# RM-Zhang/SGCDet

Hardware: AMD Instinct MI355X
Metric: scenes/sec (40-view ScanNet volume) at 1/2/4/8 MI355X; mAP@0.25 parity (higher is better)
Workload: dtype f32 (neck/head conv: 3xbf16-split MFMA, fp32 accumulate, ~1e-5 of fp32; wide 3x3x3 stride-1 layers through a Winograd F(2,3) transform along z: <= 2e-5 of the tensor scale per layer against the direct fp32 convolution); 1 GPU; cfg2_scannet: 40 views x 256 ch, images 256x320, FPN maps 64x80/32x40/16x20, D=12, voxels 40x40x16, top-k [800, 6400], neck 3-scale -> ScanNetImVoxelHeadV2; occupancy=predicted, masked_tail=False, input_layout=nchw, scenes_in_flight_per_gpu=4, launch=one hipGraph replay per scene (device-side pair counts, no host read-back)

## Files before the change

### include/sgcdet_amd_image.h

```cpp
#ifndef SGCDET_AMD_IMAGE_H_
#define SGCDET_AMD_IMAGE_H_

#include "sgcdet_amd.h"

#ifdef __cplusplus
extern "C" {
#endif

#define SGC_CONV2D_RELU 1
#define SGC_CONV2D_RELU_AFTER_ADD 2

int sgc_conv2d_nhwc_ex_bf16x3(const float *x, const uint16_t *w_hi, const uint16_t *w_lo, const float *scale,
                              const float *shift, const float *residual_or_null, float *y, int N, int H, int W, int Cin,
                              int Cout, int ksize, int stride, int transposed, int flags, int ldy, int col0, int ldr,
                              int softmax_cols, sgc_stream_t stream);
int sgc_conv2d_nhwc_ex_supported(int N, int H, int W, int Cin, int Cout, int ksize, int stride, int transposed, int ldy,
                                 int col0, int ldr , int softmax_cols);

int sgc_conv2d_stem7_bf16x3(const float *img, const uint16_t *w_hi, const uint16_t *w_lo, const float *scale,
                            const float *shift, float *y, int N, int H, int W, int relu, sgc_stream_t stream);

int sgc_nchw_to_nhwc_padc(const float *src, float *dst, int N, int C, int H, int W, int Cp, sgc_stream_t stream);

#ifdef __cplusplus
}
#endif
#endif
```

### sgcdet_amd/_abi.py

```python
import ctypes as C

_p = C.c_void_p
_i = C.c_int
_f = C.c_float
_d = C.c_double

SIGNATURES = {
    "sgc_depth_score_forward": [_p, _p, _p, _p, _p] + [_i] * 7 + [_p],
    "sgc_wms_forward": [_p, _p, _p, _p, _p, _p, _p] + [_i] * 7 + [_p],
    "sgc_wms_backward": [_p] * 11 + [_i] * 7 + [_p],
    "sgc_depth_score_backward": [_p] * 7 + [_i] * 7 + [_p],
    "sgc_dfa3d_forward": [_p] * 8 + [_i] * 9 + [_p],
    "sgc_dfa3d_backward": [_p] * 11 + [_i] * 9 + [_p],
    "sgc_dfa3d_forward_items": [_p] * 9 + [_i] * 9 + [_p],
    "sgc_dfa3d_backward_items": [_p] * 12 + [_i] * 9 + [_p],
    "sgc_dfa3d_backward_binned": [_p] * 11 + [_i] * 13 + [_p],
    "sgc_project_points": [_p] * 6 + [_i, _i, _f, _f, _f, _f, _p],
    "sgc_compact_pairs": [_p, _i, _i] + [_p] * 9 + [_p],
    "sgc_pairs_geometry_sample": [_p] * 7 + [_i] * 9 + [_p],
    "sgc_pairs_geometry_linear_bf16x3": [_p] * 11 + [_i] * 10 + [_p],
    "sgc_pairs_deform_gather": [_p] * 9 + [_i] * 12 + [_p],
    "sgc_depth_pairs": [_p, _p] + [_i] * 5 + [_p],
    "sgc_bin_pairs": [_p] * 9 + [_i] * 7 + [_p],
    "sgc_pairs_deform_gather_tiled": [_p, _i] + [_p] * 6 + [_i] * 15 + [_p],
# ... 61 lines not shown
    "sgc_linear_rows_blockdiag_supported": (C.c_int, [_i] * 3),
    "sgc_pairs_geometry_linear_workspace_bytes": (C.c_int64, [_i]),
}

TRAIN_SIGNATURES = {
    "sgc_plane_sweep_corr_backward": [_p] * 7 + [C.c_int64] + [_i] * 6 + [_p],
    "sgc_grad_sqnorm_batch": [_p, _i, _i, _p, _p, _p],
    "sgc_adamw_step_batch": [_p, _i, _i, _p, _i, _p, _f, _p],
    "sgc_head_loss_forward": [_p, _i] + [_p] * 4 + [_i] * 4 + [_d] * 5 + [_p] * 5 + [C.c_int64, _p],
    "sgc_head_loss_finalize": [_p, C.c_int64, _p, _i, _p] + [_d] * 3 + [_p] * 3,
    "sgc_head_loss_scale_grads": [_p, _p, _p] + [_i] * 3 + [_p] * 5,
}

TRAIN_INTROSPECTION = {
    "sgc_plane_sweep_corr_backward_workspace_bytes": (C.c_int64, [_i] * 5),
    "sgc_grad_sqnorm_batch_workspace_bytes": (C.c_int64, [_i]),
    "sgc_head_loss_workspace_bytes": (C.c_int64, [_i] * 2),
}

IMAGE_SIGNATURES = {
    "sgc_conv2d_nhwc_ex_bf16x3": [_p] * 7 + [_i] * 13 + [_p],
    "sgc_conv2d_stem7_bf16x3": [_p] * 6 + [_i] * 4 + [_p],
    "sgc_nchw_to_nhwc_padc": [_p, _p] + [_i] * 5 + [_p],
}

IMAGE_INTROSPECTION = {
    "sgc_conv2d_nhwc_ex_supported": (C.c_int, [_i] * 12),
}

CONV2D_RELU, CONV2D_RELU_AFTER_ADD = 1, 2


class OptimGroup(C.Structure):
    _fields_ = [("lr", C.c_double), ("weight_decay", C.c_double), ("beta1", C.c_double), ("beta2", C.c_double), ("eps", C.c_double)]


OPTIM_ITEM_BYTES = 64
HEAD_LOSS_LEVEL_BYTES = 64
HEAD_LOSS_MAX_SCALES = 4

ABI_VERSION = 4


class SgcError(RuntimeError):
    """Raised when an entry point returns a negative status."""


class Library:

    def __init__(self, path, train=False, image=False):
# ... 40 lines not shown
```

### sgcdet_amd/csrc/rows_gemm.hip

```cpp
#include <stdlib.h>

#include "conv_common.hpp"
#include "tuning.hpp"
#include "mma.hpp"
#include "diag.hpp"

namespace sgc {



struct RowsGemmParams {
  const float *x;
  int64_t ldx;
  const __bf16 *w_hi, *w_lo;
  const float *scale, *shift;
  const float *residual;
  void *y;
  const int32_t *m_dev;
  int M, N;
  int relu;
  int hm_S, hm_cm, hm_bf16;
  int ncg;
  int diag;
  unsigned long long *stamps;
  int64_t y_bytes;
  float *zero_row;
  const float *gw;
  const int32_t *go;
  int64_t x_rows;
};

constexpr int RG_ROWS = 32;

typedef unsigned int u32x4 __attribute__((ext_vector_type(4)));
constexpr unsigned RG_OOB = 0xfffffff0u;

template <int K, int NW, int DEPTH, int EPI, int NP = 3, bool GATHER = false>
__global__ __launch_bounds__(NW * 64, 2) void rows_gemm_bf16x3_kernel(const RowsGemmParams p) {
  static_assert(!GATHER || (DEPTH == 1 && EPI == 0), "the gather form runs the lockstep schedule with the plain epilogue");
  constexpr int NT = NW * 64;
  constexpr int KS = K / 16;
  constexpr int K4 = K / 4;
  constexpr int CH = RG_ROWS * K4 / NT;
  constexpr int PITCH = K + 8;
  constexpr int PLANE = RG_ROWS * PITCH;
  static_assert(RG_ROWS * K4 % NT == 0, "tile must deal evenly");
  extern __shared__ __attribute__((aligned(16))) unsigned char rg_smem[];
  __bf16 *lds = reinterpret_cast<__bf16 *>(rg_smem);

  const int tid = threadIdx.x, lane = tid & 63, wid = tid >> 6;
  const int fr = lane & 31, fh = lane >> 5;
  if (p.zero_row && blockIdx.x == 0)
    for (int c = tid; c < p.N; c += NT) p.zero_row[c] = 0.f;
  const int Mrows = p.m_dev ? min(p.M, *p.m_dev) : p.M;
  const int ntiles = (Mrows + RG_ROWS - 1) / RG_ROWS;
  const int xcd = blockIdx.x & 7, loc = blockIdx.x >> 3;
  const int cg = loc % p.ncg, stripe = (loc / p.ncg) * 8 + xcd, nstripes = gridDim.x / p.ncg;
  if (stripe >= ntiles) return;
  const int col = (cg * NW + wid) * 32 + fr;

  const __amdgpu_buffer_rsrc_t xr = __builtin_amdgcn_make_buffer_rsrc(
      const_cast<float *>(p.x), 0, (p.diag & 2) ? 0 : (int)(unsigned)((int64_t)(GATHER ? p.x_rows : Mrows) * p.ldx * 4), 0x00020000);
  const __amdgpu_buffer_rsrc_t gwr = __builtin_amdgcn_make_buffer_rsrc(const_cast<float *>(GATHER ? p.gw : p.x), 0,
                                                                        GATHER ? (int)(unsigned)((int64_t)Mrows * 16) : 0, 0x00020000);
  const __amdgpu_buffer_rsrc_t gor = __builtin_amdgcn_make_buffer_rsrc(const_cast<int32_t *>(GATHER ? p.go : (const int32_t *)p.x), 0,
                                                                        GATHER ? (int)(unsigned)((int64_t)Mrows * 16) : 0, 0x00020000);
  const __amdgpu_buffer_rsrc_t yr = __builtin_amdgcn_make_buffer_rsrc(
      p.y, 0, (p.diag & 1) ? 0 : (int)(unsigned)((EPI == 1 || EPI == 3) ? p.y_bytes : (int64_t)Mrows * p.N * 4), 0x00020000);
  const __amdgpu_buffer_rsrc_t rr = __builtin_amdgcn_make_buffer_rsrc(
      const_cast<float *>(EPI == 2 ? p.residual : p.x), 0, (int)(unsigned)(EPI == 2 ? (int64_t)Mrows * p.N * 4 : 0), 0x00020000);

  bf16x8 bh[KS], bl[KS];
  {
    const __bf16 *wh = p.w_hi + (int64_t)col * K + fh * 8, *wl = p.w_lo + (int64_t)col * K + fh * 8;
#pragma unroll
    for (int kk = 0; kk < KS; ++kk) {
      bh[kk] = *reinterpret_cast<const bf16x8 *>(wh + kk * 16);
      if constexpr (NP == 3) bl[kk] = *reinterpret_cast<const bf16x8 *>(wl + kk * 16);
    }
  }
  const float sc = p.scale ? p.scale[col] : 1.f, sh = p.shift ? p.shift[col] : 0.f;
  const bool relu = p.relu != 0, relu1 = p.relu == 1, relu2 = p.relu == 2;

  constexpr bool STAG = DEPTH == 0;
  static_assert(!STAG || NW == 8, "the staggered form pairs waves w and w + 4 of an 8-wave workgroup");
  constexpr int NTL = STAG ? NT / 2 : NT, RL = STAG ? RG_ROWS / 2 : RG_ROWS;
  static_assert(NTL % K4 == 0 && RL * K4 / NTL == CH, "chunks of a thread must share their column");
  const int late = STAG ? __builtin_amdgcn_readfirstlane(wid >> 2) : 0;
  const int tl = STAG ? (tid & (NTL - 1)) : tid;
  const int ld_row = tl / K4 + late * RL, ld_c4 = tl % K4;
  constexpr int TV = GATHER ? 4 * CH + CH : CH;
  auto load_tile = [&](int t, float4 (&ra)[TV]) {
    int ldx4 = (int)p.ldx * 4;
    asm volatile("" : "+s"(ldx4));
    if constexpr (GATHER) {
#pragma unroll
      for (int i = 0; i < CH; ++i) {
        const unsigned doff = t < ntiles ? (unsigned)(t * RG_ROWS + ld_row + i * (NTL / K4)) * 16u : RG_OOB;
        const u32x4 o = __builtin_amdgcn_raw_buffer_load_b128(gor, doff, 0, 0);
        const u32x4 w = __builtin_amdgcn_raw_buffer_load_b128(gwr, doff, 0, 0);
        ra[4 * CH + i] = make_float4(__uint_as_float(w[0]), __uint_as_float(w[1]), __uint_as_float(w[2]), __uint_as_float(w[3]));
#pragma unroll
        for (int k = 0; k < 4; ++k) {
          const u32x4 v = __builtin_amdgcn_raw_buffer_load_b128(xr, o[k] * (unsigned)ldx4 + ld_c4 * 16, 0, 0);
          ra[4 * i + k] = make_float4(__uint_as_float(v[0]), __uint_as_float(v[1]), __uint_as_float(v[2]), __uint_as_float(v[3]));
        }
      }
      return;
    }
    const unsigned base = t < ntiles ? (unsigned)(t * RG_ROWS + ld_row) * (unsigned)ldx4 + ld_c4 * 16 : RG_OOB;
#pragma unroll
    for (int i = 0; i < CH; ++i) {
      const u32x4 v = __builtin_amdgcn_raw_buffer_load_b128(xr, t < ntiles ? base + i * (NTL / K4) * ldx4 : RG_OOB, 0, 0);
      ra[i] = make_float4(__uint_as_float(v[0]), __uint_as_float(v[1]), __uint_as_float(v[2]), __uint_as_float(v[3]));
    }
  };
  auto split_tile = [&](const float4 (&ra)[TV], int buf) {
    __bf16 *a_hi = lds + buf * 2 * PLANE, *a_lo = a_hi + PLANE;
#pragma unroll
    for (int i = 0; i < CH; ++i) {
      const int row = ld_row + i * (NTL / K4), c4 = ld_c4;
      float v[4];
      if constexpr (GATHER) {
        const float wk[4] = {ra[4 * CH + i].x, ra[4 * CH + i].y, ra[4 * CH + i].z, ra[4 * CH + i].w};
        v[0] = v[1] = v[2] = v[3] = 0.f;
#pragma unroll
        for (int k = 0; k < 4; ++k) {
          v[0] = __builtin_fmaf(wk[k], ra[4 * i + k].x, v[0]); v[1] = __builtin_fmaf(wk[k], ra[4 * i + k].y, v[1]);
          v[2] = __builtin_fmaf(wk[k], ra[4 * i + k].z, v[2]); v[3] = __builtin_fmaf(wk[k], ra[4 * i + k].w, v[3]);
        }
      } else {
        v[0] = ra[i].x; v[1] = ra[i].y; v[2] = ra[i].z; v[3] = ra[i].w;
      }
      bf16x4 h, l;
#pragma unroll
      for (int e = 0; e < 4; ++e) {
        const __bf16 hb = op_hi<NP>(v[e]);
        h[e] = hb;
        l[e] = op_lo<NP>(v[e], hb);
      }
      *reinterpret_cast<bf16x4 *>(a_hi + row * PITCH + c4 * 4) = h;
// ... 405 lines not shown
  {
    static const bool diag_ok = getenv("SGC_DIAG") && atoi(getenv("SGC_DIAG")) == 1;
    p.diag = diag_ok ? g_tune_rows_diag : 0;
  }
  RG_STAMP_BIND(p);
  const int nw = (N % 256 == 0) ? 8 : 4;
  p.ncg = N / (nw * 32);
  const int cap_tiles = ceil_div(M, RG_ROWS);
  const int per_cu = nw == 8 ? 1 : 2;
  int stripes = device_cus() * per_cu / p.ncg;
  if (g_tune_rows_cu_pct > 0 && g_tune_rows_cu_pct < 100) stripes = stripes * g_tune_rows_cu_pct / 100;
  if (stripes > cap_tiles) stripes = cap_tiles;
  stripes = (stripes + 7) / 8 * 8;
  const int grid = stripes * p.ncg;
  const int depth = nw == 8 ? g_tune_rows_depth : 1;
  if (K == 256) {
    if (nw == 8) return depth == 0 ? launch_rows_gemm<256, 8, 0>(p, grid, st) : depth == 2 ? launch_rows_gemm<256, 8, 2>(p, grid, st) : launch_rows_gemm<256, 8, 1>(p, grid, st);
    return launch_rows_gemm<256, 4, 1>(p, grid, st);
  }
  if (nw == 8) return depth == 0 ? launch_rows_gemm<128, 8, 0>(p, grid, st) : depth == 2 ? launch_rows_gemm<128, 8, 2>(p, grid, st) : launch_rows_gemm<128, 8, 1>(p, grid, st);
  return launch_rows_gemm<128, 4, 1>(p, grid, st);
}

}

#if defined(SGC_RG_STAMPS)
extern "C" void sgc_diag_rows_stamp_buffer(unsigned long long *buf) { sgc::g_rows_stamp_buf = buf; }
#endif
```

### sgcdet_amd/plugin/conv_plan.py

```python
import os

import torch

from .. import ext

_PAD = 32

CONV_MODE = "bf16x3"
CONV_PRODUCTS = 3


def set_conv_mode(mode):
    global CONV_MODE, CONV_PRODUCTS
    if mode not in ("bf16x3", "f32", "bf16", "fp16"):
        raise ValueError(mode)
    CONV_MODE = "bf16x3" if mode in ("bf16", "fp16") else mode
    CONV_PRODUCTS = {"bf16": 1, "fp16": 2}.get(mode, 3)
    import torch
    if torch.cuda.is_available():
        ext.ops().lib.call("sgc_set_conv_products", CONV_PRODUCTS)


WINOGRAD_Z = {"0": False, "1": True}.get(os.environ.get("SGC_WINOGRAD_Z", ""), "auto")
WINOGRAD_Z_MIN_CH = int(os.environ.get("SGC_WINOGRAD_Z_MIN_CH", "256"))
# ... 268 lines not shown
        self.w_hi, self.w_lo = ext.ops().split_operand(wp)
        self.shift = torch.zeros(cout_p, dtype=torch.float32, device=w.device)
        if bias is not None:
            self.shift[:cout] = bias.detach().float()
        self.cout, self.cout_p = cout, cout_p

    def __call__(self, x, extra_zero_row=False, count=None):
        M = x.shape[0]
        if CONV_MODE == "bf16x3" and self.cout_p == self.cout:
            return ext.ops().linear_rows_bf16x3(x, self.w_hi, self.w_lo, self.shift, count=count, useful=self.useful,
                                                zero_tail=bool(extra_zero_row) and M > 0)
        if count is not None:
            raise NotImplementedError("device-side row counts need the bf16x3 path and out_features % 4 == 0")
        if CONV_MODE == "bf16x3":
            y, _ = ext.ops().conv3d_cl_bf16x3(x, self.w_hi, self.w_lo, (M, 1, 1), 1, 1, False, None, self.shift)
        else:
            y, _ = ext.ops().conv3d_cl(x, self.wt, (M, 1, 1), 1, 1, False, None, self.shift)
        return y if self.cout_p == self.cout else y[:, :self.cout]

    def headmajor(self, x, N, S, M, out_dtype=torch.float32):
        if CONV_MODE != "bf16x3" or self.cout_p != self.cout:
            raise NotImplementedError("head-major output needs the bf16x3 path and out_features % 4 == 0")
        return ext.ops().linear_rows_headmajor_bf16x3(x, self.w_hi, self.w_lo, self.shift, N, S, M, out_dtype=out_dtype)
```

### sgcdet_amd/plugin/voxformer.py

```python
import copy
import math
import warnings

import torch
import torch.nn as nn
import torch.nn.functional as F

from ..mmcv_lite import (ATTENTION, TRANSFORMER, TRANSFORMER_LAYER, TRANSFORMER_LAYER_SEQUENCE,
                         BaseModule, ModuleList, TransformerLayerSequence,
                         build_attention, build_feedforward_network, build_norm_layer,
                         build_transformer_layer_sequence, constant_init, xavier_init)
from ..functions import MultiScale3DDeformableAttnFunction_fp32
from .. import ext
from .conv_plan import BlockDiagSpec, LinearSpec, cached_plan, module_fingerprint


def _ops():
    return ext.ops()


TILED_GATHER = dict(enabled=True, min_pixels=2048, storage="f32",
                    cm32=dict(bin=(16, 22), halo=(3, 3), depth_in_lds=False),
                    cm16=dict(bin=(16, 22), halo=(3, 3), depth_in_lds=True))


GEO_LINEAR_FUSED = __import__("os").environ.get("SGC_GEO_LINEAR", "1") != "0"

TRAIN_BWD_TILED = dict(enabled=True, bin=(8, 22), halo=(2, 2))


def _tiled_env_overrides():
    import os
    if "SGC_TILED" in os.environ:
        TILED_GATHER["enabled"] = os.environ["SGC_TILED"] != "0"
    if os.environ.get("SGC_STORAGE") in ("f32", "bf16"):
        TILED_GATHER["storage"] = os.environ["SGC_STORAGE"]
    spec = os.environ.get("SGC_TRAIN_BWD")
    if spec == "0":
        TRAIN_BWD_TILED["enabled"] = False
    elif spec:
        bw, bh, hx, hy = (int(v) for v in spec.split(","))
        TRAIN_BWD_TILED.update(enabled=True, bin=(bw, bh), halo=(hx, hy))
    for key in ("cm32", "cm16"):
        spec = os.environ.get("SGC_TILED_" + key.upper())
        if spec:
            bw, bh, hx, hy, dl = (int(v) for v in spec.split(","))
            TILED_GATHER[key] = dict(bin=(bw, bh), halo=(hx, hy), depth_in_lds=bool(dl))


# ... 209 lines not shown
        wqo = w[:C] @ self.output_proj.weight.detach().double()
        bqo = w[:C] @ self.output_proj.bias.detach().double() + b[:C]
        wk, wv, bv = w[C:2 * C], w[2 * C:], b[2 * C:]
        scale = (1.0 / hd) ** 0.5
        wqp = torch.cat([scale * wk[h * hd:(h + 1) * hd].t() @ wqo[h * hd:(h + 1) * hd] for h in range(Hn)], 0)
        bqp = torch.cat([scale * wk[h * hd:(h + 1) * hd].t() @ bqo[h * hd:(h + 1) * hd] for h in range(Hn)], 0)
        wbd = torch.zeros((C, Hn * C), dtype=torch.float64, device=w.device)
        for h in range(Hn):
            wbd[h * hd:(h + 1) * hd, h * C:(h + 1) * C] = wv[h * hd:(h + 1) * hd]
        vg = None
        if self.projected_query_blockdiag and BlockDiagSpec.supported(Hn, C, hd):
            vg = BlockDiagSpec(wv.view(Hn, hd, C).float(), bv.float())
        return dict(qp=LinearSpec(wqp.float(), bqp.float()), vbd=LinearSpec(wbd.float(), bv.float(), useful=1.0 / Hn), vbd_g=vg)

    def _use_projected_query(self, gemm, n_views, n_rows_cap=0):
        if gemm is None or gemm.get("qp") is None or self.projected_query is False:
            return False
        if 2 * n_rows_cap * self.attention_pooling.num_heads * self.embed_dims * 4 > self.projected_query_max_bytes:
            return False
        if not _ops().view_attend_pq_supported(n_views, self.embed_dims, self.attention_pooling.num_heads):
            return False
        return self.projected_query is True or n_views >= self.projected_query_min_views

    def _forward_pairs(self, query, feat, dist, ref_cam, mask_u8, H, W, zero_query=False, static_counts=False, want_ctx=False):
        ops = _ops()
        C = self.embed_dims
        N, Nq = mask_u8.shape
        from .conv_plan import CONV_MODE
        use_mfma = self.deformable_attn and self.inter_view_aggregation == "attn" and C % 32 == 0
        pc = ops.compact_pairs(mask_u8)
        if static_counts:
            if not (use_mfma and CONV_MODE == "bf16x3"):
                raise NotImplementedError("static_counts needs the bf16x3 GEMM path (attn aggregation, C % 32 == 0)")
            n_pairs, n_valid = -1, Nq
            totals, pairs_cnt, valid_cnt = pc["totals"], pc["totals"][0:1], pc["totals"][1:2]
        else:
            n_pairs, n_valid, _, _ = pc["totals"].tolist()
            totals = pairs_cnt = valid_cnt = None
        if n_pairs == 0:
            if want_ctx:
                return torch.zeros((1, C), dtype=feat.dtype, device=feat.device), pc["row_of"]
            out = torch.zeros((1, Nq, C), dtype=feat.dtype, device=feat.device)
            return out if zero_query else self.dropout(out) + query
        pair_cam, pair_q = pc["pair_cam"], pc["pair_q"]
        gemm = self._gemm_plan() if use_mfma else None
        da = self.deformable_attention
        S = feat.shape[1]
        Cm = C // da.num_heads
        tiled = None
        if (self.deformable_attn and use_mfma and CONV_MODE in ("bf16x3", "f32") and TILED_GATHER["enabled"] and da.num_levels == 1
                and da.num_points == 4 and Cm in (16, 32) and TILED_GATHER["min_pixels"] <= H * W < 32767
                and dist.shape[-1] >= 2):
            tiled = TILED_GATHER["cm32" if Cm == 32 else "cm16"]
            bw, bh = min(tiled["bin"][0], W), min(tiled["bin"][1], H)
            pc = ops.bin_pairs(ref_cam, pc, H, W, bw, bh)
            pair_q = pc["pair_q"]
        fuse_geo = (GEO_LINEAR_FUSED and self.deformable_attn and not self.geo_residual and use_mfma and CONV_MODE == "bf16x3"
                    and da.num_levels == 1 and ops.pairs_geometry_linear_supported(C, da.num_heads * da.num_points * 4, N, S))
        geo = None if fuse_geo else ops.pairs_geometry_sample(feat, dist, ref_cam, pair_cam, pair_q, n_pairs, H, W, totals=totals)

        def raw_projection(spec):
            if fuse_geo:
                return ops.pairs_geometry_linear(feat, dist, ref_cam, pair_cam, pair_q, n_pairs, H, W, spec.w_hi, spec.w_lo, spec.shift,
                                                 totals=totals)
            return spec(geo, count=pairs_cnt)

        if self.deformable_attn:
            if da.num_levels != 1:
                raise NotImplementedError("pair-list path supports num_levels == 1 (all SGCDet configs)")
            if tiled is not None:
                if CONV_MODE == "bf16x3":
                    value = gemm["value"].headmajor(feat.view(N * S, C), N, S, da.num_heads,
                                                    out_dtype=torch.bfloat16 if TILED_GATHER["storage"] == "bf16" else torch.float32)
                else:
                    value = gemm["value"](feat.view(N * S, C)).view(N, S, da.num_heads, Cm).permute(0, 2, 1, 3).contiguous()
                raw = raw_projection(gemm["raw_hm"])
                if not self.geo_residual:
                    del geo
                dist_g = dist.to(torch.bfloat16) if value.dtype == torch.bfloat16 else dist
                per_pair = ops.pairs_deform_gather_tiled(value, dist_g, pc["pair_ref"], pc["bin_offset"], raw, H, W,
                                                         da.num_points, bw, bh, tiled["halo"][0], tiled["halo"][1],
                                                         head_shift=gemm["head_shift"], max_shift=gemm["max_shift"],
                                                         depth_in_lds=tiled["depth_in_lds"])
                if n_pairs >= 0:
                    per_pair = per_pair[:n_pairs]
            else:
                zero_row = use_mfma and CONV_MODE == "bf16x3"
                value = gemm["value"](feat.view(N * S, C), extra_zero_row=zero_row) if use_mfma else da.value_proj(feat)
                raw = raw_projection(gemm["raw"]) if use_mfma else da.raw_projection(geo)
                if not self.geo_residual:
                    del geo
                per_pair = ops.pairs_deform_gather(value.view(N, S, da.num_heads, C // da.num_heads), dist,
                                                   ref_cam, raw, pair_cam, pair_q, n_pairs, H, W,
                                                   da.num_heads, da.num_points, totals=totals,
# ... 143 lines not shown
        pooled = self.output_proj(pooled)
        if self.inter_view_aggregation == "attn":
            pooled, _ = self.attention_pooling(pooled[None], valid_slots, valid_slots, ~valid_mask.t())
            pooled = pooled[0]
        out = torch.zeros((1, Nq, C), dtype=feat.dtype, device=feat.device)
        out = out.index_put((torch.zeros_like(valid_index), valid_index), pooled)
        return self.dropout(out) + query

    def _depth_inputs(self, value_dpt_dist, reference_points_cam, N, S, Nq, feat):
        return value_dpt_dist.reshape(N, S, -1), reference_points_cam.reshape(N, Nq, 3)

    def forward(self, query, key, value, residual=None, query_pos=None, key_padding_mask=None,
                reference_points=None, spatial_shapes=None, reference_points_cam=None, bev_mask=None,
                level_start_index=None, value_dpt_dist=None, flag="encoder", **kwargs):
        if value is None:
            value = key
        if query_pos is not None:
            query = query + query_pos
        bs, Nq, C = query.shape
        assert bs == 1
        N, S = value.shape[0], value.shape[1]
        feat = value.reshape(N, S, C)
        dist, ref_cam = self._depth_inputs(value_dpt_dist, reference_points_cam, N, S, Nq, feat)
        if torch.is_grad_enabled() and (query.requires_grad or feat.requires_grad or dist.requires_grad
                                        or any(p.requires_grad for p in self.parameters())):
            if self.train_pair_list:
                return self._forward_pairs_train(query, feat, dist, ref_cam, bev_mask.reshape(N, Nq), spatial_shapes, level_start_index,
                                                 spatial_hw=kwargs.get("spatial_hw"))
            return self._forward_reference_layout(query, feat, dist, ref_cam, bev_mask.reshape(N, Nq).bool(), spatial_shapes,
                                                  level_start_index)
        if spatial_shapes.shape[0] != 1:
            raise NotImplementedError("pair-list path supports one feature level per call (all SGCDet configs)")
        hw = kwargs.get("spatial_hw")
        if hw is None:
            hw = tuple(int(v) for v in spatial_shapes[0].tolist())
        mask_u8 = bev_mask.reshape(N, Nq)
        mask_u8 = mask_u8 if mask_u8.dtype == torch.uint8 else mask_u8.to(torch.uint8)
        return self._forward_pairs(query, feat.contiguous(), dist.contiguous(), ref_cam.contiguous(),
                                   mask_u8.contiguous(), hw[0], hw[1], zero_query=bool(kwargs.get("zero_query")),
                                   static_counts=bool(kwargs.get("static_counts")), want_ctx=bool(kwargs.get("want_ctx")))


@ATTENTION.register_module()
class DeformCrossAttention(DeformCrossAttention_DFA3D):
    geo_residual = True

    def _depth_inputs(self, value_dpt_dist, reference_points_cam, N, S, Nq, feat):
        ref = reference_points_cam.reshape(N, Nq, -1)
        if ref.shape[-1] == 2:
            ref = torch.cat([ref, ref.new_full((N, Nq, 1), 0.5)], -1)
        else:
            ref = ref.clone()
            ref[..., 2] = 0.5
        ones = self.__dict__.get("_unit_depth")
        if ones is None or ones.shape != (N, S, 1) or ones.device != feat.device or ones.dtype != feat.dtype:
            ones = self.__dict__["_unit_depth"] = feat.new_ones((N, S, 1))
        return ones, ref


@TRANSFORMER_LAYER.register_module()
class MyCustomBaseTransformerLayer(BaseModule):

    def __init__(self, attn_cfgs=None, ffn_cfgs=None, operation_order=None, norm_cfg=dict(type="LN"),
# ... 336 lines not shown
                    feats.append(feat[0].flatten(2).permute(0, 2, 1))
                else:
                    f_rows = _channels_last_rows(feat[0], h, w) if feat.dtype == torch.float32 else None
                    feats.append(f_rows if f_rows is not None else ops.nchw_to_nhwc_crop(feat[0].float(), h, w))
            elif torch.is_grad_enabled() and (feat.requires_grad or dpt.requires_grad):
                if feat.is_cuda and feat.dtype == torch.float32 and dpt.dtype == torch.float32:
                    from ..functions import NchwToRowsFunction
                    feats.append(NchwToRowsFunction.apply(feat[0]))
                    dists.append(NchwToRowsFunction.apply(dpt[0]))
                else:
                    feats.append(feat[0].flatten(2).permute(0, 2, 1))
                    dists.append(dpt[0].flatten(2).permute(0, 2, 1))
            else:
                f_rows = _channels_last_rows(feat[0], h, w) if feat.dtype == torch.float32 else None
                d_rows = _channels_last_rows(dpt[0], h, w) if dpt.dtype == torch.float32 else None
                if f_rows is not None and (d_rows is None or f_rows.shape[1] != d_rows.shape[1]):
                    d = ops.nchw_to_nhwc_crop(dpt[0].float(), h, w)
                    if f_rows.shape[1] == h * w:
                        d_rows = d
                    else:
                        d_rows = d.new_empty((n_cam, f_rows.shape[1], d.shape[2]))
                        d_rows[:, :h * w] = d
                elif f_rows is None or d_rows is None:
                    f_rows = ops.nchw_to_nhwc_crop(feat[0].float(), h, w)
                    d_rows = ops.nchw_to_nhwc_crop(dpt[0].float(), h, w)
                feats.append(f_rows)
                dists.append(d_rows)
        feat_flatten = feats[0] if len(feats) == 1 else torch.cat(feats, 1)
        dist_flatten = None if not dists else (dists[0] if len(dists) == 1 else torch.cat(dists, 1))
        spatial_shapes, level_start_index = self._shape_tensors(tuple(shapes), queries.device)
        pos = None
        if bev_pos is not None:
            pos = bev_pos.flatten(2).permute(2, 0, 1)[flat_idx]
        return self.encoder(queries, feat_flatten.unsqueeze(2), feat_flatten.unsqueeze(2),
                            value_dpt_dist=None if dist_flatten is None else dist_flatten.unsqueeze(2), ref_3d=sel_ref[None, None],
                            bev_pos=pos, spatial_shapes=spatial_shapes, level_start_index=level_start_index,
                            img_meta=img_meta, prev_bev=None, spatial_hw=shapes[0] if len(shapes) == 1 else None,
                            ref_sel=ref_sel, **kwargs)


@TRANSFORMER.register_module()
class PerceptionTransformer(PerceptionTransformer_DFA3D):

    def get_vox_features(self, mlvl_feats, bev_queries, ref_3d, vox_coords, unmasked_idx, bev_pos=None,
                         prev_bev=None, img_meta=None, **kwargs):
        kwargs.pop("mlvl_dpt_dists", None)
        return super().get_vox_features(mlvl_feats, bev_queries, ref_3d, vox_coords, unmasked_idx, bev_pos=bev_pos,
# ... 2 lines not shown
```

### sgcdet_amd/tensor_api.py

```python
import torch


def _stream_ptr(device_type, index=None):
    if device_type == "cuda":
        if index is not None and hasattr(torch._C, "_cuda_getCurrentRawStream"):
            return torch._C._cuda_getCurrentRawStream(index)
        return torch.cuda.current_stream().cuda_stream
    return None


class TensorOps:
    def __init__(self, library, device_type):
        self.lib = library
        self.device_type = device_type
        self.event_log = None
        self.event_names = None

    def _check(self, **tensors):
        dev = None
        for name, t in tensors.items():
            if t is None:
                continue
            if not isinstance(t, torch.Tensor):
                raise RuntimeError(f"{name} must be a tensor")
# ... 9 lines not shown
                raise RuntimeError(f"{name} is on {t.device}, expected {dev}")
        return dev

    @staticmethod
    def _f32(**tensors):
        for name, t in tensors.items():
            if t is not None and t.dtype != torch.float32:
                raise RuntimeError(f"{name} must be float32 (got {t.dtype})")

    @staticmethod
    def _i64(**tensors):
        for name, t in tensors.items():
            if t.dtype != torch.int64:
                raise RuntimeError(f"{name} must be int64 (got {t.dtype})")

    @staticmethod
    def _i32(**tensors):
        for name, t in tensors.items():
            if t is not None and t.dtype != torch.int32:
                raise RuntimeError(f"{name} must be int32 (got {t.dtype})")

    n_calls = 0

    def _call(self, name, *args, _meta=None):
        self.n_calls += 1
        ptrs = [a.data_ptr() if isinstance(a, torch.Tensor) else a for a in args]
        if self.device_type == "cuda":
            dev = next(a.device for a in args if isinstance(a, torch.Tensor))
            idx = dev.index if dev.index is not None else torch.cuda.current_device()
            if idx != torch.cuda.current_device():
                with torch.cuda.device(dev):
                    return self._call(name, *args, _meta=_meta)
            if self.event_log is None or (self.event_names is not None and name not in self.event_names):
                return self.lib.call(name, *ptrs, _stream_ptr("cuda", idx))
            e0 = torch.cuda.Event(enable_timing=True)
            e1 = torch.cuda.Event(enable_timing=True)
            e0.record()
            rc = self.lib.call(name, *ptrs, _stream_ptr("cuda", idx))
            e1.record()
            self.event_log.append((name, _meta or {}, e0, e1))
            return rc
        return self.lib.call(name, *ptrs, None)

    def depth_score_forward(self, dist, shapes3, lsi, loc3):
        self._check(value=dist, value_spatial_shapes=shapes3, value_level_start_index=lsi,
                    sampling_locations=loc3)
        self._f32(value=dist, sampling_locations=loc3)
        self._i64(value_spatial_shapes=shapes3, value_level_start_index=lsi)
        B, S, M, D = dist.shape
        _, Q, M2, L, P, three = loc3.shape
        if M2 != M or three != 3 or shapes3.shape != (L, 3) or loc3.shape[0] != B:
            raise RuntimeError("ms_depth_score_sample_forward: inconsistent shapes")
        score = torch.empty((B, Q, M, L, P, 4), dtype=dist.dtype, device=dist.device)
        self._call("sgc_depth_score_forward", dist, shapes3, lsi, loc3, score, B, S, M, D, L, Q, P)
        return score

    def wms_forward(self, value, shapes2, lsi, loc2, attn, score):
        self._check(value=value, value_spatial_shapes=shapes2, value_level_start_index=lsi,
                    sampling_locations=loc2, attention_weights=attn, depth_scores=score)
        self._f32(value=value, sampling_locations=loc2, attention_weights=attn, depth_scores=score)
        self._i64(value_spatial_shapes=shapes2, value_level_start_index=lsi)
        B, S, M, Cm = value.shape
        _, Q, _, L, P, two = loc2.shape
# ... 308 lines not shown
        self._call("sgc_pairs_deform_gather_tiled", value_hm, int(value_hm.dtype == torch.bfloat16), dist, pair_ref,
                   bin_offset, raw_hm, head_shift, out,
                   N, H, W, M, Cm, D, P, S, bin_w, bin_h, halo_x, halo_y, int(max_shift[0]), int(max_shift[1]),
                   int(bool(depth_in_lds)),
                   _meta=dict(N=N, H=H, W=W, C=M * Cm, D=D, M=M, P=P, n_pairs=rows, bin=(bin_w, bin_h), halo=(halo_x, halo_y),
                              value_bytes=value_hm.element_size(), depth_bytes=dist.element_size()))
        return out

    def linear_rows_headmajor_bf16x3(self, x, w_hi, w_lo, shift, N, S, M, out_dtype=torch.float32):
        self._check(x=x, w_hi=w_hi, w_lo=w_lo, shift=shift)
        self._f32(x=x, shift=shift)
        rows, Cin = x.shape
        Cout = w_hi.shape[-2]
        if rows != N * S or Cout % M or w_hi.shape[-1] != Cin or w_hi.dtype != torch.bfloat16 or w_lo.dtype != torch.bfloat16:
            raise RuntimeError("linear_rows_headmajor_bf16x3: inconsistent shapes")
        Cm = Cout // M
        if out_dtype not in (torch.float32, torch.bfloat16):
            raise RuntimeError("linear_rows_headmajor_bf16x3: out_dtype must be float32 or bfloat16")
        y = torch.empty((N, M, S, Cm), dtype=out_dtype, device=x.device)
        self._call("sgc_linear_rows_headmajor_bf16x3", x, w_hi, w_lo, shift, y, int(out_dtype == torch.bfloat16), N, S, Cin, M, Cm,
                   _meta=dict(V=rows, Cin=Cin, Cout=Cout, taps=1, OV=rows))
        return y

    def view_mean(self, feat, slot, valid_index, n_valid, count=None):
        self._check(feat=feat, slot=slot, valid_index=valid_index, count=count)
        self._f32(feat=feat)
        self._i32(slot=slot, valid_index=valid_index, count=count)
        N, Nq = slot.shape
        Cc = feat.shape[1]
        mean = torch.empty((n_valid, Cc), dtype=torch.float32, device=feat.device)
        if n_valid == 0:
            return mean
        self._call("sgc_view_mean", feat, slot, valid_index, mean, N, Nq, Cc, count, n_valid)
        return mean

    def view_attend_backward(self, q, kv, slot, valid_index, heads, ctx, grad_ctx):
        self._check(q=q, kv=kv, slot=slot, valid_index=valid_index, ctx=ctx, grad_ctx=grad_ctx)
        self._f32(q=q, kv=kv, ctx=ctx, grad_ctx=grad_ctx)
        self._i32(slot=slot, valid_index=valid_index)
        N, Nq = slot.shape
        n_valid, Cc = q.shape
        gq = torch.zeros_like(q)
        gkv = torch.zeros_like(kv)
        if n_valid:
            self._call("sgc_view_attend_backward", q, kv, slot, valid_index, ctx, grad_ctx, gq, gkv, N, Nq, Cc, heads, n_valid)
        return gq, gkv
# ... 22 lines not shown
        N, Nq = slot.shape
        n_valid, HC = qp.shape
        Cc = x.shape[1]
        if HC != heads * Cc:
            raise RuntimeError("view_attend_pq: qp must be [n_valid, heads * C]")
        s = torch.empty_like(qp)
        if n_valid == 0:
            return s
        self._call("sgc_view_attend_pq", qp, x, slot, valid_index, s, N, Nq, Cc, heads, count, n_valid)
        return s

    def scatter_rows(self, rows, idx, vol, idx2=None, count=None):
        self._check(rows=rows, idx=idx, vol=vol, idx2=idx2, count=count)
        self._f32(rows=rows, vol=vol)
        self._i32(idx=idx, idx2=idx2, count=count)
        n, Cc = rows.shape
        if vol.shape[-1] != Cc:
            raise RuntimeError("scatter_rows: channel mismatch")
        if n == 0:
            return vol
        self._call("sgc_scatter_rows", rows, idx, idx2, vol, count, n, Cc)
        return vol

    def nchw_to_nhwc_crop(self, src, H, W):
        if src.dim() != 4:
            raise RuntimeError("nchw_to_nhwc_crop expects [N,C,H,W]")
        N, Cc, h_in, w_in = src.shape
        if H > h_in or W > w_in:
            raise RuntimeError("nchw_to_nhwc_crop: crop larger than the map")
        st = src.stride()
        step = st[3] if w_in > 1 else 1
        viewable = False
        if step >= 1 and h_in > 1 and st[2] % step == 0:
            Ws = st[2] // step
            Hs = st[1] // Ws if Ws > 0 and st[1] % Ws == 0 else 0
            viewable = (Ws >= (w_in - 1) * step + 1 and Hs >= (h_in - 1) * step + 1 and st[1] == Hs * Ws
                        and (N == 1 or st[0] == Cc * Hs * Ws))
        if not viewable:
            src = src.contiguous()
            Hs, Ws, step = h_in, w_in, 1
        if src.device.type != self.device_type:
            raise RuntimeError(f"src must be a {self.device_type} tensor")
        self._f32(src=src)
        dst = torch.empty((N, H * W, Cc), dtype=torch.float32, device=src.device)
        self._call("sgc_nchw_to_nhwc_crop", src, dst, N, Cc, Hs, Ws, H, W, step)
        return dst

    def nhwc_to_nchw_pad(self, rows, H, W, Hd=None, Wd=None):
        self._check(rows=rows)
        self._f32(rows=rows)
        N, S, Cc = rows.shape
        Hd, Wd = H if Hd is None else Hd, W if Wd is None else Wd
        if S != H * W or Hd < H or Wd < W:
            raise RuntimeError("nhwc_to_nchw_pad: inconsistent shapes")
        dst = torch.empty((N, Cc, Hd, Wd), dtype=torch.float32, device=rows.device)
        self._call("sgc_nhwc_to_nchw_pad", rows, dst, N, Cc, H, W, Hd, Wd)
        return dst

    @staticmethod
    def split_bf16(w):
        hi = w.to(torch.bfloat16)
        lo = (w - hi.float()).to(torch.bfloat16)
        return hi.contiguous(), lo.contiguous()

    @staticmethod
    def split_f16(w):
        hi = w.clamp(-65504.0, 65504.0).to(torch.float16).view(torch.bfloat16)
# ... 696 lines not shown
```

Measured before the change: 525.8 scenes/sec.

## Fuse NCHW-to-NHWC crop into head-major value projection GEMM

The inference path used to transpose the NCHW FPN feature plane into NHWC rows and then run the head-major value projection over those rows. It now postpones the transpose: the rows GEMM kernel gains an NCHW mode that gathers 8-channel blocks directly from the strided plane, splits them to bf16 hi/lo, and optionally writes the NHWC rows as a side output for the other consumers (geometry sampling). This drops one standalone transpose kernel and one read of the feature plane. In exchange the GEMM issues strided scalar loads, and the hand-over goes through a deferred 'feat_nchw' state that is allowed only under no_grad.

```diff
diff --git a/include/sgcdet_amd_image.h b/include/sgcdet_amd_image.h
--- a/include/sgcdet_amd_image.h
+++ b/include/sgcdet_amd_image.h
@@ -22,6 +22,11 @@
 
 int sgc_nchw_to_nhwc_padc(const float *src, float *dst, int N, int C, int H, int W, int Cp, sgc_stream_t stream);
 
+int sgc_linear_rows_headmajor_nchw_bf16x3(const float *x, const uint16_t *w_hi, const uint16_t *w_lo, const float *shift, void *y,
+                                          int y_bf16, float *rows_out_or_null, int N, int C, int Hs, int Ws, int H, int W, int M,
+                                          int Cm, sgc_stream_t stream);
+int sgc_linear_rows_headmajor_nchw_supported(int C, int Cout, int Cm, int N, int Hs, int Ws, int H, int W);
+
 #ifdef __cplusplus
 }
 #endif
diff --git a/sgcdet_amd/_abi.py b/sgcdet_amd/_abi.py
--- a/sgcdet_amd/_abi.py
+++ b/sgcdet_amd/_abi.py
@@ -107,10 +107,12 @@
     "sgc_conv2d_nhwc_ex_bf16x3": [_p] * 7 + [_i] * 13 + [_p],
     "sgc_conv2d_stem7_bf16x3": [_p] * 6 + [_i] * 4 + [_p],
     "sgc_nchw_to_nhwc_padc": [_p, _p] + [_i] * 5 + [_p],
+    "sgc_linear_rows_headmajor_nchw_bf16x3": [_p] * 5 + [_i, _p] + [_i] * 8 + [_p],
 }
 
 IMAGE_INTROSPECTION = {
     "sgc_conv2d_nhwc_ex_supported": (C.c_int, [_i] * 12),
+    "sgc_linear_rows_headmajor_nchw_supported": (C.c_int, [_i] * 8),
 }
 
 CONV2D_RELU, CONV2D_RELU_AFTER_ADD = 1, 2
diff --git a/sgcdet_amd/csrc/rows_gemm.hip b/sgcdet_amd/csrc/rows_gemm.hip
--- a/sgcdet_amd/csrc/rows_gemm.hip
+++ b/sgcdet_amd/csrc/rows_gemm.hip
@@ -28,6 +28,11 @@
   const float *gw;
   const int32_t *go;
   int64_t x_rows;
+  int nchw_W, nchw_Ws;
+  unsigned nchw_magic_w;
+  int64_t nchw_plane;
+  int64_t x_bytes;
+  float *rows_out;
 };
 
 constexpr int RG_ROWS = 32;
@@ -35,9 +40,10 @@
 typedef unsigned int u32x4 __attribute__((ext_vector_type(4)));
 constexpr unsigned RG_OOB = 0xfffffff0u;
 
-template <int K, int NW, int DEPTH, int EPI, int NP = 3, bool GATHER = false>
+template <int K, int NW, int DEPTH, int EPI, int NP = 3, bool GATHER = false, bool NCHW = false>
 __global__ __launch_bounds__(NW * 64, 2) void rows_gemm_bf16x3_kernel(const RowsGemmParams p) {
   static_assert(!GATHER || (DEPTH == 1 && EPI == 0), "the gather form runs the lockstep schedule with the plain epilogue");
+  static_assert(!NCHW || (DEPTH == 1 && !GATHER && (EPI == 1 || EPI == 3)), "the NCHW form is the head-major value projection, lockstep");
   constexpr int NT = NW * 64;
   constexpr int KS = K / 16;
   constexpr int K4 = K / 4;
@@ -60,7 +66,7 @@
   const int col = (cg * NW + wid) * 32 + fr;
 
   const __amdgpu_buffer_rsrc_t xr = __builtin_amdgcn_make_buffer_rsrc(
-      const_cast<float *>(p.x), 0, (p.diag & 2) ? 0 : (int)(unsigned)((int64_t)(GATHER ? p.x_rows : Mrows) * p.ldx * 4), 0x00020000);
+      const_cast<float *>(p.x), 0, (p.diag & 2) ? 0 : (int)(unsigned)(NCHW ? p.x_bytes : (int64_t)(GATHER ? p.x_rows : Mrows) * p.ldx * 4), 0x00020000);
   const __amdgpu_buffer_rsrc_t gwr = __builtin_amdgcn_make_buffer_rsrc(const_cast<float *>(GATHER ? p.gw : p.x), 0,
                                                                         GATHER ? (int)(unsigned)((int64_t)Mrows * 16) : 0, 0x00020000);
   const __amdgpu_buffer_rsrc_t gor = __builtin_amdgcn_make_buffer_rsrc(const_cast<int32_t *>(GATHER ? p.go : (const int32_t *)p.x), 0,
@@ -69,6 +75,9 @@
       p.y, 0, (p.diag & 1) ? 0 : (int)(unsigned)((EPI == 1 || EPI == 3) ? p.y_bytes : (int64_t)Mrows * p.N * 4), 0x00020000);
   const __amdgpu_buffer_rsrc_t rr = __builtin_amdgcn_make_buffer_rsrc(
       const_cast<float *>(EPI == 2 ? p.residual : p.x), 0, (int)(unsigned)(EPI == 2 ? (int64_t)Mrows * p.N * 4 : 0), 0x00020000);
+  const __amdgpu_buffer_rsrc_t cr = __builtin_amdgcn_make_buffer_rsrc(
+      NCHW && p.rows_out ? (void *)p.rows_out : (void *)p.y, 0, (NCHW && p.rows_out && !(p.diag & 1)) ? (int)(unsigned)((int64_t)Mrows * K * 4) : 0,
+      0x00020000);
 
   bf16x8 bh[KS], bl[KS];
   {
@@ -90,7 +99,33 @@
   const int tl = STAG ? (tid & (NTL - 1)) : tid;
   const int ld_row = tl / K4 + late * RL, ld_c4 = tl % K4;
   constexpr int TV = GATHER ? 4 * CH + CH : CH;
+  constexpr int NB = CH / 2, CBS = NT / 32;
+  static_assert(!NCHW || (CH % 2 == 0 && NB * CBS * 8 == K), "NCHW deal: whole 8-channel blocks");
+  const int px = tid & 31, cb0 = tid >> 5;
+  unsigned cp_off = RG_OOB;
   auto load_tile = [&](int t, float4 (&ra)[TV]) {
+    if constexpr (NCHW) {
+      const int m0 = t * RG_ROWS;
+      int cam = m0 / p.hm_S, s = m0 - cam * p.hm_S + px;
+      if (s >= p.hm_S) { s -= p.hm_S; ++cam; }
+      const bool live = m0 + px < Mrows;
+      if (!live) { cam = (Mrows - 1) / p.hm_S; s = Mrows - 1 - cam * p.hm_S; }
+      const int h = (int)__umulhi((unsigned)s, p.nchw_magic_w), w = s - h * p.nchw_W;
+      int plane4 = (int)p.nchw_plane * 4;
+      asm volatile("" : "+s"(plane4));
+      const unsigned base = (unsigned)(cam * K + cb0 * 8) * (unsigned)plane4 + (unsigned)(h * p.nchw_Ws + w) * 4u;
+      cp_off = live ? (unsigned)(m0 + px) * (unsigned)(K * 4) + cb0 * 32 : RG_OOB;
+#pragma unroll
+      for (int b = 0; b < NB; ++b) {
+        const unsigned off = base + (unsigned)(b * CBS * 8) * (unsigned)plane4;
+        float v[8];
+#pragma unroll
+        for (int j = 0; j < 8; ++j) v[j] = __uint_as_float(__builtin_amdgcn_raw_buffer_load_b32(xr, off, j * plane4, 0));
+        ra[2 * b] = make_float4(v[0], v[1], v[2], v[3]);
+        ra[2 * b + 1] = make_float4(v[4], v[5], v[6], v[7]);
+      }
+      return;
+    }
     int ldx4 = (int)p.ldx * 4;
     asm volatile("" : "+s"(ldx4));
     if constexpr (GATHER) {
@@ -117,6 +152,29 @@
   };
   auto split_tile = [&](const float4 (&ra)[TV], int buf) {
     __bf16 *a_hi = lds + buf * 2 * PLANE, *a_lo = a_hi + PLANE;
+    if constexpr (NCHW) {
+#pragma unroll
+      for (int b = 0; b < NB; ++b) {
+        const float v[8] = {ra[2 * b].x, ra[2 * b].y, ra[2 * b].z, ra[2 * b].w, ra[2 * b + 1].x, ra[2 * b + 1].y, ra[2 * b + 1].z, ra[2 * b + 1].w};
+        bf16x8 h, l;
+#pragma unroll
+        for (int e = 0; e < 8; ++e) {
+          const __bf16 hb = op_hi<NP>(v[e]);
+          h[e] = hb;
+          l[e] = op_lo<NP>(v[e], hb);
+        }
+        const int c = (cb0 + b * CBS) * 8;
+        *reinterpret_cast<bf16x8 *>(a_hi + px * PITCH + c) = h;
+        if constexpr (NP == 3) *reinterpret_cast<bf16x8 *>(a_lo + px * PITCH + c) = l;
+        if (p.rows_out) {
+          const unsigned o = cp_off == RG_OOB ? RG_OOB : cp_off + (unsigned)(b * CBS * 32);
+          const unsigned o2 = cp_off == RG_OOB ? RG_OOB : o + 16u;
+          __builtin_amdgcn_raw_buffer_store_b128(u32x4{__float_as_uint(v[0]), __float_as_uint(v[1]), __float_as_uint(v[2]), __float_as_uint(v[3])}, cr, o, 0, 0);
+          __builtin_amdgcn_raw_buffer_store_b128(u32x4{__float_as_uint(v[4]), __float_as_uint(v[5]), __float_as_uint(v[6]), __float_as_uint(v[7])}, cr, o2, 0, 0);
+        }
+      }
+      return;
+    }
 #pragma unroll
     for (int i = 0; i < CH; ++i) {
       const int row = ld_row + i * (NTL / K4), c4 = ld_c4;
@@ -568,6 +626,71 @@
   return launch_rows_gemm<128, 4, 1>(p, grid, st);
 }
 
+bool rows_gemm_nchw_supported(int C, int Cout, int Cm, int N, int Hs, int Ws, int H, int W) {
+  if (N <= 0 || H <= 0 || W <= 0 || H > Hs || W > Ws || Cout != C) return false;
+  const int64_t S = (int64_t)H * W;
+  if (S * W >= (1ll << 31) || (int64_t)N * C * Hs * Ws * 4 >= (int64_t)RG_OOB) return false;
+  return rows_gemm_supported(C, Cout, Cm, (int)S, (int64_t)N * S, C);
+}
+
+template <int K, int NW, int EPI>
+static int launch_rows_gemm_nchw(const RowsGemmParams &p, int grid, hipStream_t st) {
+  constexpr int smem = 2 * 2 * RG_ROWS * (K + 8) * (int)sizeof(uint16_t);
+  with_products(g_conv_products, [&](auto np) {
+    static std::atomic<uint64_t> attr_done{0};
+    ensure_dynamic_lds((const void *)rows_gemm_bf16x3_kernel<K, NW, 1, EPI, np(), false, true>, smem, attr_done);
+    hipLaunchKernelGGL((rows_gemm_bf16x3_kernel<K, NW, 1, EPI, np(), false, true>), dim3(grid), dim3(NW * 64), smem, st, p);
+  });
+  return check_launch("rows_gemm_bf16x3_kernel (nchw)");
+}
+
+int rows_gemm_nchw_launch(const float *x, const uint16_t *w_hi, const uint16_t *w_lo, const float *shift, void *y, int y_bf16,
+                          float *rows_out, int N, int C, int Hs, int Ws, int H, int W, int Cm, hipStream_t st) {
+  RowsGemmParams p = {};
+  p.x = x; p.ldx = C;
+  p.w_hi = reinterpret_cast<const __bf16 *>(w_hi); p.w_lo = reinterpret_cast<const __bf16 *>(w_lo);
+  p.shift = shift; p.y = y;
+  p.M = N * H * W; p.N = C;
+  p.hm_S = H * W; p.hm_cm = Cm; p.hm_bf16 = y_bf16;
+  p.y_bytes = (int64_t)p.M * p.N * (y_bf16 ? 2 : 4);
+  p.nchw_W = W; p.nchw_Ws = Ws; p.nchw_plane = (int64_t)Hs * Ws;
+  p.nchw_magic_w = (unsigned)((1ull << 32) / (unsigned)W + 1);
+  p.x_bytes = (int64_t)N * C * Hs * Ws * 4;
+  p.rows_out = rows_out;
+  {
+    static const bool diag_ok = getenv("SGC_DIAG") && atoi(getenv("SGC_DIAG")) == 1;
+    p.diag = diag_ok ? g_tune_rows_diag : 0;
+  }
+  const int nw = C == 256 ? 8 : 4;
+  p.ncg = 1;
+  const int cap_tiles = ceil_div(p.M, RG_ROWS);
+  int stripes = device_cus() * (nw == 8 ? 1 : 2);
+  if (g_tune_rows_cu_pct > 0 && g_tune_rows_cu_pct < 100) stripes = stripes * g_tune_rows_cu_pct / 100;
+  if (stripes > cap_tiles) stripes = cap_tiles;
+  stripes = (stripes + 7) / 8 * 8;
+  if (C == 256) return y_bf16 ? launch_rows_gemm_nchw<256, 8, 3>(p, stripes, st) : launch_rows_gemm_nchw<256, 8, 1>(p, stripes, st);
+  return y_bf16 ? launch_rows_gemm_nchw<128, 4, 3>(p, stripes, st) : launch_rows_gemm_nchw<128, 4, 1>(p, stripes, st);
+}
+
+}
+
+extern "C" int sgc_linear_rows_headmajor_nchw_supported(int C, int Cout, int Cm, int N, int Hs, int Ws, int H, int W) {
+  return sgc::rows_gemm_nchw_supported(C, Cout, Cm, N, Hs, Ws, H, W) ? 1 : 0;
+}
+
+extern "C" int sgc_linear_rows_headmajor_nchw_bf16x3(const float *x, const uint16_t *w_hi, const uint16_t *w_lo, const float *shift,
+                                                     void *y, int y_bf16, float *rows_out_or_null, int N, int C, int Hs, int Ws, int H,
+                                                     int W, int M, int Cm, sgc_stream_t stream) {
+  using namespace sgc;
+  if (!x || !w_hi || !w_lo || !y) return set_error(SGC_EINVAL, "sgc_linear_rows_headmajor_nchw_bf16x3: null pointer");
+  if (M <= 0 || Cm <= 0 || Cm % 4) return set_error(SGC_EINVAL, "sgc_linear_rows_headmajor_nchw_bf16x3: bad size (Cm %% 4 == 0 required)");
+  if (((uintptr_t)x | (uintptr_t)w_hi | (uintptr_t)w_lo | (uintptr_t)y | (uintptr_t)rows_out_or_null) & 15)
+    return set_error(SGC_EINVAL, "sgc_linear_rows_headmajor_nchw_bf16x3: pointers must be 16-byte aligned");
+  if (!rows_gemm_nchw_supported(C, M * Cm, Cm, N, Hs, Ws, H, W))
+    return set_error(SGC_EUNSUP, "sgc_linear_rows_headmajor_nchw_bf16x3: needs Cout == C in {128, 256}, Cm | 128, a crop of >= 32 pixels "
+                                 "inside the plane and a plane below 4 GiB (got C %d, Cout %d, Cm %d, crop %d x %d of %d x %d)",
+                     C, M * Cm, Cm, H, W, Hs, Ws);
+  return rows_gemm_nchw_launch(x, w_hi, w_lo, shift, y, y_bf16 ? 1 : 0, rows_out_or_null, N, C, Hs, Ws, H, W, Cm, (hipStream_t)stream);
 }
 
 #if defined(SGC_RG_STAMPS)
diff --git a/sgcdet_amd/plugin/conv_plan.py b/sgcdet_amd/plugin/conv_plan.py
--- a/sgcdet_amd/plugin/conv_plan.py
+++ b/sgcdet_amd/plugin/conv_plan.py
@@ -314,3 +314,9 @@
         if CONV_MODE != "bf16x3" or self.cout_p != self.cout:
             raise NotImplementedError("head-major output needs the bf16x3 path and out_features % 4 == 0")
         return ext.ops().linear_rows_headmajor_bf16x3(x, self.w_hi, self.w_lo, self.shift, N, S, M, out_dtype=out_dtype)
+
+    def headmajor_nchw(self, plane, H, W, M, out_dtype=torch.float32, rows_out=None):
+        if CONV_MODE != "bf16x3" or self.cout_p != self.cout:
+            raise NotImplementedError("head-major output needs the bf16x3 path and out_features % 4 == 0")
+        return ext.ops().linear_rows_headmajor_nchw(plane, H, W, self.w_hi, self.w_lo, self.shift, M, out_dtype=out_dtype,
+                                                    rows_out=rows_out)
diff --git a/sgcdet_amd/plugin/voxformer.py b/sgcdet_amd/plugin/voxformer.py
--- a/sgcdet_amd/plugin/voxformer.py
+++ b/sgcdet_amd/plugin/voxformer.py
@@ -25,6 +25,7 @@
 
 
 GEO_LINEAR_FUSED = __import__("os").environ.get("SGC_GEO_LINEAR", "1") != "0"
+NCHW_INPLACE = __import__("os").environ.get("SGC_NCHW_INPLACE", "1") != "0"
 
 TRAIN_BWD_TILED = dict(enabled=True, bin=(8, 22), halo=(2, 2))
 
@@ -280,7 +281,8 @@
             return False
         return self.projected_query is True or n_views >= self.projected_query_min_views
 
-    def _forward_pairs(self, query, feat, dist, ref_cam, mask_u8, H, W, zero_query=False, static_counts=False, want_ctx=False):
+    def _forward_pairs(self, query, feat, dist, ref_cam, mask_u8, H, W, zero_query=False, static_counts=False, want_ctx=False,
+                       feat_nchw=None):
         ops = _ops()
         C = self.embed_dims
         N, Nq = mask_u8.shape
@@ -313,6 +315,16 @@
             bw, bh = min(tiled["bin"][0], W), min(tiled["bin"][1], H)
             pc = ops.bin_pairs(ref_cam, pc, H, W, bw, bh)
             pair_q = pc["pair_q"]
+        value = None
+        if feat_nchw is not None and not feat_nchw["done"]:
+            plane = feat_nchw["plane"]
+            if (tiled is not None and CONV_MODE == "bf16x3" and S == H * W and gemm["value"].cout_p == gemm["value"].cout
+                    and ops.linear_rows_headmajor_nchw_supported(plane, H, W, C, da.num_heads)):
+                value = gemm["value"].headmajor_nchw(plane, H, W, da.num_heads, rows_out=feat,
+                                                     out_dtype=torch.bfloat16 if TILED_GATHER["storage"] == "bf16" else torch.float32)
+            else:
+                ops.nchw_to_nhwc_crop(plane, H, W, out=feat)
+            feat_nchw["done"] = True
         fuse_geo = (GEO_LINEAR_FUSED and self.deformable_attn and not self.geo_residual and use_mfma and CONV_MODE == "bf16x3"
                     and da.num_levels == 1 and ops.pairs_geometry_linear_supported(C, da.num_heads * da.num_points * 4, N, S))
         geo = None if fuse_geo else ops.pairs_geometry_sample(feat, dist, ref_cam, pair_cam, pair_q, n_pairs, H, W, totals=totals)
@@ -327,7 +339,9 @@
             if da.num_levels != 1:
                 raise NotImplementedError("pair-list path supports num_levels == 1 (all SGCDet configs)")
             if tiled is not None:
-                if CONV_MODE == "bf16x3":
+                if value is not None:
+                    pass
+                elif CONV_MODE == "bf16x3":
                     value = gemm["value"].headmajor(feat.view(N * S, C), N, S, da.num_heads,
                                                     out_dtype=torch.bfloat16 if TILED_GATHER["storage"] == "bf16" else torch.float32)
                 else:
@@ -517,8 +531,11 @@
         N, S = value.shape[0], value.shape[1]
         feat = value.reshape(N, S, C)
         dist, ref_cam = self._depth_inputs(value_dpt_dist, reference_points_cam, N, S, Nq, feat)
+        feat_nchw = kwargs.get("feat_nchw")
         if torch.is_grad_enabled() and (query.requires_grad or feat.requires_grad or dist.requires_grad
                                         or any(p.requires_grad for p in self.parameters())):
+            if feat_nchw is not None:
+                raise RuntimeError("the deferred NCHW hand-over is an inference route (get_vox_features defers under no_grad only)")
             if self.train_pair_list:
                 return self._forward_pairs_train(query, feat, dist, ref_cam, bev_mask.reshape(N, Nq), spatial_shapes, level_start_index,
                                                  spatial_hw=kwargs.get("spatial_hw"))
@@ -533,7 +550,8 @@
         mask_u8 = mask_u8 if mask_u8.dtype == torch.uint8 else mask_u8.to(torch.uint8)
         return self._forward_pairs(query, feat.contiguous(), dist.contiguous(), ref_cam.contiguous(),
                                    mask_u8.contiguous(), hw[0], hw[1], zero_query=bool(kwargs.get("zero_query")),
-                                   static_counts=bool(kwargs.get("static_counts")), want_ctx=bool(kwargs.get("want_ctx")))
+                                   static_counts=bool(kwargs.get("static_counts")), want_ctx=bool(kwargs.get("want_ctx")),
+                                   feat_nchw=feat_nchw)
 
 
 @ATTENTION.register_module()
@@ -916,7 +934,12 @@
                         d_rows = d.new_empty((n_cam, f_rows.shape[1], d.shape[2]))
                         d_rows[:, :h * w] = d
                 elif f_rows is None or d_rows is None:
-                    f_rows = ops.nchw_to_nhwc_crop(feat[0].float(), h, w)
+                    if (NCHW_INPLACE and not torch.is_grad_enabled() and len(mlvl_feats) == 1 and feat.is_cuda
+                            and feat.dtype == torch.float32 and ops.nchw_plane_in_place(feat[0])):
+                        f_rows = torch.empty((n_cam, h * w, c), dtype=torch.float32, device=feat.device)
+                        kwargs["feat_nchw"] = dict(plane=feat[0], done=False)
+                    else:
+                        f_rows = ops.nchw_to_nhwc_crop(feat[0].float(), h, w)
                     d_rows = ops.nchw_to_nhwc_crop(dpt[0].float(), h, w)
                 feats.append(f_rows)
                 dists.append(d_rows)
diff --git a/sgcdet_amd/tensor_api.py b/sgcdet_amd/tensor_api.py
--- a/sgcdet_amd/tensor_api.py
+++ b/sgcdet_amd/tensor_api.py
@@ -55,7 +55,10 @@
 
     n_calls = 0
 
-    def _call(self, name, *args, _meta=None):
+    def _call_as(self, log_name, name, *args, _meta=None):
+        return self._call(name, *args, _meta=_meta, _log_name=log_name)
+
+    def _call(self, name, *args, _meta=None, _log_name=None):
         self.n_calls += 1
         ptrs = [a.data_ptr() if isinstance(a, torch.Tensor) else a for a in args]
         if self.device_type == "cuda":
@@ -63,15 +66,16 @@
             idx = dev.index if dev.index is not None else torch.cuda.current_device()
             if idx != torch.cuda.current_device():
                 with torch.cuda.device(dev):
-                    return self._call(name, *args, _meta=_meta)
-            if self.event_log is None or (self.event_names is not None and name not in self.event_names):
+                    return self._call(name, *args, _meta=_meta, _log_name=_log_name)
+            log_name = _log_name or name
+            if self.event_log is None or (self.event_names is not None and log_name not in self.event_names):
                 return self.lib.call(name, *ptrs, _stream_ptr("cuda", idx))
             e0 = torch.cuda.Event(enable_timing=True)
             e1 = torch.cuda.Event(enable_timing=True)
             e0.record()
             rc = self.lib.call(name, *ptrs, _stream_ptr("cuda", idx))
             e1.record()
-            self.event_log.append((name, _meta or {}, e0, e1))
+            self.event_log.append((log_name, _meta or {}, e0, e1))
             return rc
         return self.lib.call(name, *ptrs, None)
 
@@ -426,6 +430,58 @@
                    _meta=dict(V=rows, Cin=Cin, Cout=Cout, taps=1, OV=rows))
         return y
 
+    @staticmethod
+    def _nchw_plane(src):
+        N, Cc, h_in, w_in = src.shape
+        st = src.stride()
+        step = st[3] if w_in > 1 else 1
+        if step >= 1 and h_in > 1 and st[2] % step == 0:
+            Ws = st[2] // step
+            Hs = st[1] // Ws if Ws > 0 and st[1] % Ws == 0 else 0
+            if (Ws >= (w_in - 1) * step + 1 and Hs >= (h_in - 1) * step + 1 and st[1] == Hs * Ws
+                    and (N == 1 or st[0] == Cc * Hs * Ws)):
+                return Hs, Ws, step
+        return None
+
+    def nchw_plane_in_place(self, src):
+        if src.dim() != 4 or src.dtype != torch.float32:
+            return False
+        plane = self._nchw_plane(src)
+        return plane is not None and plane[2] == 1
+
+    def linear_rows_headmajor_nchw_supported(self, src, H, W, Cout, M):
+        if src.dim() != 4 or src.dtype != torch.float32 or src.device.type != self.device_type or Cout % M:
+            return False
+        N, Cc, h_in, w_in = src.shape
+        plane = self._nchw_plane(src)
+        if plane is None or plane[2] != 1 or H > h_in or W > w_in or src.data_ptr() % 16:
+            return False
+        return bool(self.lib._dll.sgc_linear_rows_headmajor_nchw_supported(int(Cc), int(Cout), int(Cout // M), int(N), int(plane[0]),
+                                                                            int(plane[1]), int(H), int(W)))
+
+    def linear_rows_headmajor_nchw(self, src, H, W, w_hi, w_lo, shift, M, out_dtype=torch.float32, rows_out=None):
+        self._check(w_hi=w_hi, w_lo=w_lo, shift=shift, rows_out=rows_out)
+        self._f32(shift=shift, rows_out=rows_out)
+        Cout = w_hi.shape[-2]
+        if not self.linear_rows_headmajor_nchw_supported(src, H, W, Cout, M):
+            raise RuntimeError("linear_rows_headmajor_nchw: unsupported plane / shape (ask linear_rows_headmajor_nchw_supported)")
+        N, Cc = src.shape[:2]
+        Hs, Ws, _ = self._nchw_plane(src)
+        S = H * W
+        if w_hi.shape[-1] != Cc or w_hi.dtype != torch.bfloat16 or w_lo.dtype != torch.bfloat16 or w_lo.shape != w_hi.shape:
+            raise RuntimeError("linear_rows_headmajor_nchw: inconsistent weight planes")
+        if out_dtype not in (torch.float32, torch.bfloat16):
+            raise RuntimeError("linear_rows_headmajor_nchw: out_dtype must be float32 or bfloat16")
+        if rows_out is not None and (tuple(rows_out.shape) != (N, S, Cc) or not rows_out.is_contiguous()):
+            raise RuntimeError("linear_rows_headmajor_nchw: rows_out must be contiguous [N, H*W, C]")
+        Cm = Cout // M
+        y = torch.empty((N, M, S, Cm), dtype=out_dtype, device=src.device)
+        rows = N * S
+        self._call_as("sgc_linear_rows_headmajor_bf16x3", "sgc_linear_rows_headmajor_nchw_bf16x3", src, w_hi, w_lo, shift, y,
+                      int(out_dtype == torch.bfloat16), rows_out, N, Cc, Hs, Ws, H, W, M, Cm,
+                      _meta=dict(V=rows, Cin=Cc, Cout=Cout, taps=1, OV=rows))
+        return y
+
     def view_mean(self, feat, slot, valid_index, n_valid, count=None):
         self._check(feat=feat, slot=slot, valid_index=valid_index, count=count)
         self._f32(feat=feat)
@@ -494,27 +550,27 @@
         self._call("sgc_scatter_rows", rows, idx, idx2, vol, count, n, Cc)
         return vol
 
-    def nchw_to_nhwc_crop(self, src, H, W):
+    def nchw_to_nhwc_crop(self, src, H, W, out=None):
         if src.dim() != 4:
             raise RuntimeError("nchw_to_nhwc_crop expects [N,C,H,W]")
         N, Cc, h_in, w_in = src.shape
         if H > h_in or W > w_in:
             raise RuntimeError("nchw_to_nhwc_crop: crop larger than the map")
-        st = src.stride()
-        step = st[3] if w_in > 1 else 1
-        viewable = False
-        if step >= 1 and h_in > 1 and st[2] % step == 0:
-            Ws = st[2] // step
-            Hs = st[1] // Ws if Ws > 0 and st[1] % Ws == 0 else 0
-            viewable = (Ws >= (w_in - 1) * step + 1 and Hs >= (h_in - 1) * step + 1 and st[1] == Hs * Ws
-                        and (N == 1 or st[0] == Cc * Hs * Ws))
-        if not viewable:
+        plane = self._nchw_plane(src)
+        if plane is None:
             src = src.contiguous()
             Hs, Ws, step = h_in, w_in, 1
+        else:
+            Hs, Ws, step = plane
         if src.device.type != self.device_type:
             raise RuntimeError(f"src must be a {self.device_type} tensor")
         self._f32(src=src)
-        dst = torch.empty((N, H * W, Cc), dtype=torch.float32, device=src.device)
+        if out is None:
+            dst = torch.empty((N, H * W, Cc), dtype=torch.float32, device=src.device)
+        else:
+            dst = out
+            if tuple(dst.shape) != (N, H * W, Cc) or dst.dtype != torch.float32 or not dst.is_contiguous() or dst.device != src.device:
+                raise RuntimeError("nchw_to_nhwc_crop: out must be contiguous fp32 [N, H*W, C] on the device of src")
         self._call("sgc_nchw_to_nhwc_crop", src, dst, N, Cc, Hs, Ws, H, W, step)
         return dst
 
```

New measurement: 530.2 scenes/sec (median of 5 runs). Within noise of the previous version (+0.8%).
